# klutzy/suruga

Hardware: AMD Instinct MI355X
Metric: GiB/s device-resident ChaCha20-Poly1305 over 16 KiB TLS records, 1/2/4/8 GPUs (higher is better)
Workload: dtype u32

## Files before the change

suruga_amd/csrc/sg_msg.hip:

```cpp
#include "sg_internal.h"
#include "sg_msg_plan.h"

#include "sg_device.h"

namespace sg {
namespace {

using namespace dev;

constexpr uint32_t kLdsFront = 64;
constexpr uint32_t kLdsBytes = kLdsFront + 64u + kMsgTileBytes + 16u;

struct MsgKey {
    uint32_t k[8];
    uint32_t r0, r1, r2, r3;
    uint32_t s[4];
};

__device__ __forceinline__ MsgKey msg_key(const uint8_t* key, uint32_t n14, uint32_t n15) {
    MsgKey mk;
#pragma unroll
    for (int i = 0; i < 8; ++i)
        mk.k[i] = uniform((uint32_t)key[4 * i] | ((uint32_t)key[4 * i + 1] << 8) | ((uint32_t)key[4 * i + 2] << 16) |
                          ((uint32_t)key[4 * i + 3] << 24));
    uint32_t ks[16];
    chacha_block(ks, mk.k, 0u, n14, n15);
    mk.r0 = uniform(ks[0] & 0x0fffffffu);
    mk.r1 = uniform(ks[1] & 0x0ffffffcu);
    mk.r2 = uniform(ks[2] & 0x0ffffffcu);
    mk.r3 = uniform(ks[3] & 0x0ffffffcu);
#pragma unroll
    for (int i = 0; i < 4; ++i) mk.s[i] = uniform(ks[4 + i]);
    return mk;
}

__device__ __forceinline__ F26 fpow(const F26 x, const uint32_t e) {
    F26 acc = f26_one();
    if (e == 0u) return acc;
    for (int bit = 31 - __builtin_clz(e); bit >= 0; --bit) {
        acc = fmul(acc, acc);
        if ((e >> bit) & 1u) acc = fmul(acc, x);
    }
    return acc;
}

__device__ __forceinline__ F26 block_sum(const F26 x, uint32_t* red, const uint32_t lane) {
    store_f26(red + 5u * lane, x);
    __syncthreads();
    if (lane < 16u) {
        F26 a = f26_zero();
        for (uint32_t i = 0; i < 16u; ++i) a = f26_add(a, load_f26(red + 5u * (16u * lane + i)));
        store_f26(red + 5u * (256u + lane), carry1(a));
    }
    __syncthreads();
    F26 a = f26_zero();
    if (lane == 0u) {
        for (uint32_t i = 0; i < 16u; ++i) a = f26_add(a, load_f26(red + 5u * (256u + i)));
        a = carry1(a);
    }
    return a;
}

}

struct MsgParams {
    const uint8_t* key;
    const uint8_t* ad;
    const uint8_t* in;
    uint8_t* out;
    uint8_t* status;
    uint32_t* ws;
    uint64_t n, adlen;
    uint32_t n14, n15;
    sg_msg_plan plan;
};

namespace {

template <bool OPEN>
__global__ __launch_bounds__(256) void sg_msg_kernel(const MsgParams p) {
    __shared__ __attribute__((aligned(64))) uint8_t lds[kLdsBytes];
    static_assert(kLdsBytes >= 5u * 4u * (256u + 16u), "reduction space");
    const uint32_t lane = threadIdx.x;
    const MsgKey mk = msg_key(p.key, p.n14, p.n15);
    const uint32_t r0 = mk.r0, r1 = mk.r1, r2 = mk.r2, r3 = mk.r3;
    const uint32_t s1 = r1 + (r1 >> 2), s2 = r2 + (r2 >> 2), s3 = r3 + (r3 >> 2);
    const F26 r = words_to_f26(r0, r1, r2, r3, 0u);
    const F26 R = fpow(r, p.plan.tile_blocks);
    const F26 Pl = fpow(r, lane < kMsgMacLanes ? kMsgLaneBlocks * (kMsgMacLanes - 1u - lane) : 0u);
    const ChaChaPre pre = chacha_pre(mk.k, p.n14, p.n15);

    const int64_t n = (int64_t)p.n;
    const int64_t adlen = (int64_t)p.adlen;
    const int64_t P = adlen + 8;
    const int64_t L = P + n + 8;
    const int64_t TB = (int64_t)p.plan.tile_bytes;
    const uint64_t z = p.plan.zero_blocks;
    const uint64_t last = z + p.plan.mac_blocks - 1u;
    const uint32_t rem = (uint32_t)(L - 16 * ((int64_t)p.plan.mac_blocks - 1));

    const uint64_t t0 = (uint64_t)blockIdx.x * p.plan.tiles_per_group;
    uint64_t t1 = t0 + p.plan.tiles_per_group;
    if (t1 > p.plan.tiles) t1 = p.plan.tiles;

    F26 acc = f26_zero();
    for (uint64_t t = t0; t < t1; ++t) {
        const int64_t s0 = (int64_t)t * TB - 16 * (int64_t)z;
        const int64_t s1e = s0 + TB;
        const int64_t d0 = s0 - P > 0 ? s0 - P : 0;
        const int64_t d1 = s1e - P < n ? s1e - P : n;
        const uint32_t A = (uint32_t)((s0 - P) & 63);
        uint8_t* tl = lds + kLdsFront + A;

        if (d1 > d0) {
            const int64_t cb = (d0 >> 6) + (int64_t)lane;
            const int64_t boff = cb << 6;
            if (boff < d1) {
                const uint8_t* ip = p.in + boff;
                uint8_t* op = p.out + boff;
                uint8_t* lp = tl + (P + boff - s0);
                const bool al = ((((uintptr_t)ip) | ((uintptr_t)op)) & 15u) == 0u;
                const bool full = al && boff >= d0 && boff + 64 <= d1;
                u32x4 dv[4] = {};
                bool vec[4] = {full, full, full, full};
                if (full) {
#pragma unroll
                    for (int c = 0; c < 4; ++c) dv[c] = gld16(ip + 16 * c);
                } else {
#pragma unroll
                    for (int c = 0; c < 4; ++c) {
                        const int64_t co = boff + 16 * c;
                        vec[c] = al && co + 16 > d0 && co < d1 && co + 16 <= n;
                        if (vec[c]) dv[c] = gld16(ip + 16 * c);
                    }
                }
                uint32_t ks[16];
                chacha_block_pre(ks, pre, mk.k, (uint32_t)cb + 1u, p.n14, p.n15);
                if (full) {
                    u32x4 xv[4];
#pragma unroll
                    for (int c = 0; c < 4; ++c) {
                        xv[c] = dv[c] ^ u32x4{ks[4 * c], ks[4 * c + 1], ks[4 * c + 2], ks[4 * c + 3]};
                        asm volatile("" : "+v"(xv[c].x), "+v"(xv[c].y), "+v"(xv[c].z), "+v"(xv[c].w));
                    }
#pragma unroll
                    for (int c = 0; c < 4; ++c) st16(lp + 16 * c, OPEN ? dv[c] : xv[c]);
#pragma unroll
                    for (int c = 0; c < 4; ++c) gst16(op + 16 * c, xv[c]);
                } else {
#pragma unroll
                for (int c = 0; c < 4; ++c) {
                    const int64_t co = boff + 16 * c;
                    if (co + 16 <= d0 || co >= d1) continue;
                    if (vec[c]) {
                        const u32x4 d = dv[c];
                        const u32x4 x = d ^ u32x4{ks[4 * c], ks[4 * c + 1], ks[4 * c + 2], ks[4 * c + 3]};
                        st16(lp + 16 * c, OPEN ? d : x);
                        if (co >= d0 && co + 16 <= d1) {
                            gst16(op + 16 * c, x);
                        } else {
                            const uint32_t xw[4] = {x.x, x.y, x.z, x.w};
#pragma unroll
                            for (int b = 0; b < 16; ++b)
                                if (co + b >= d0 && co + b < d1) op[16 * c + b] = (uint8_t)(xw[b >> 2] >> (8 * (b & 3)));
                        }
                    } else {
                        uint8_t xb[16];
#pragma unroll
                        for (int b = 0; b < 16; ++b) xb[b] = co + b >= d0 && co + b < d1 ? ip[16 * c + b] : (uint8_t)0;
#pragma unroll
                        for (int b = 0; b < 16; ++b) {
                            if (co + b >= d0 && co + b < d1) {
                                const uint8_t y = xb[b] ^ (uint8_t)(ks[4 * c + (b >> 2)] >> (8 * (b & 3)));
                                op[16 * c + b] = y;
                                lp[16 * c + b] = OPEN ? xb[b] : y;
                            }
                        }
                    }
                }
                }
            }
        }
        if (s0 < P || s1e > P + n) {
            int64_t a = s0 > 0 ? s0 : 0, b = s1e < P ? s1e : P;
            for (int64_t s = a + lane; s < b; s += kMsgThreads)
                tl[s - s0] = s < adlen ? p.ad[s] : (uint8_t)((uint64_t)adlen >> (8 * (s - adlen)));
            a = s0 > P + n ? s0 : P + n;
            for (int64_t s = a + lane; s < s1e; s += kMsgThreads) {
                const int64_t i = s - (P + n);
                tl[s - s0] = i < 8 ? (uint8_t)((uint64_t)n >> (8 * i)) : (uint8_t)0;
            }
        }
        __syncthreads();

        if (lane < kMsgMacLanes) {
            const uint64_t vb0 = t * p.plan.tile_blocks + kMsgLaneBlocks * lane;
            const uint8_t* bp = tl + 16u * kMsgLaneBlocks * lane;
            H32 h = {0u, 0u, 0u, 0u, 0u};
#pragma unroll
            for (uint32_t j = 0; j < kMsgLaneBlocks; ++j) {
                u32x4 m = ldu16(bp + 16u * j);
                const uint64_t vb = vb0 + j;
                uint32_t pad = 1u;
                if (vb < z) {
                    m = u32x4{0u, 0u, 0u, 0u};
                    pad = 0u;
                } else if (vb == last && rem < 16u) {
                    const uint32_t fb = 1u << (8u * (rem & 3u));
                    const uint32_t fw = rem >> 2;
                    m.x |= fw == 0u ? fb : 0u;
                    m.y |= fw == 1u ? fb : 0u;
                    m.z |= fw == 2u ? fb : 0u;
                    m.w |= fw == 3u ? fb : 0u;
                    pad = 0u;
                }
                horner_step(h, m.x, m.y, m.z, m.w, pad, r0, r1, r2, r3, s1, s2, s3);
            }
            F26 f = words_to_f26(h.h0, h.h1, h.h2, h.h3, 0u);
            f.v4 += h.h4 << 24;
            const uint32_t c = f.v4 >> 26;
            f.v4 &= M26;
            f.v0 += c * 5u;
            acc = fmul_add(acc, R, f);
        }
        __syncthreads();
    }
    const F26 Hg = block_sum(fmul(acc, Pl), reinterpret_cast<uint32_t*>(lds), lane);
    if (lane == 0u) store_f26(p.ws + (uint64_t)blockIdx.x * kMsgPartialWords, Hg);
}

template <bool OPEN>
__global__ __launch_bounds__(256) void sg_msg_finish_kernel(const MsgParams p) {
    __shared__ uint32_t red[5u * (256u + 16u)];
    const uint32_t lane = threadIdx.x;
    const MsgKey mk = msg_key(p.key, p.n14, p.n15);
    const F26 R = fpow(words_to_f26(mk.r0, mk.r1, mk.r2, mk.r3, 0u), p.plan.tile_blocks);
    F26 sum = f26_zero();
    for (uint32_t g = lane; g < p.plan.groups; g += 256u) {
        const uint64_t done = (uint64_t)(g + 1u) * p.plan.tiles_per_group;
        const uint32_t after = done >= p.plan.tiles ? 0u : (uint32_t)(p.plan.tiles - done);
        sum = f26_add(sum, fmul(load_f26(p.ws + (uint64_t)g * kMsgPartialWords), fpow(R, after)));
    }
    const F26 total = block_sum(carry1(sum), red, lane);
    if (lane != 0u) return;
    uint32_t tw[4];
    tag_words(total, mk.s, tw);
    if constexpr (!OPEN) {
        uint8_t* tp = p.out + p.n;
#pragma unroll
        for (int i = 0; i < 16; ++i) tp[i] = (uint8_t)(tw[i >> 2] >> (8 * (i & 3)));
    } else {
        const uint8_t* ep = p.in + p.n;
        uint32_t diff = 0u;
#pragma unroll
        for (int i = 0; i < 16; ++i) diff |= (uint32_t)ep[i] ^ ((tw[i >> 2] >> (8 * (i & 3))) & 0xffu);
        *p.status = diff != 0u ? 1u : 0u;
    }
}

__global__ __launch_bounds__(256) void sg_msg_scrub_kernel(uint8_t* out, const uint64_t n, const uint8_t* status) {
    if (*status == 0u) return;
    uint64_t head = (16u - ((uintptr_t)out & 15u)) & 15u;
    if (head > n) head = n;
    const uint64_t nvec = (n - head) >> 4;
    const uint64_t tail0 = head + (nvec << 4);
    const uint64_t i = (uint64_t)blockIdx.x * 256u + threadIdx.x;
    const uint64_t stride = (uint64_t)gridDim.x * 256u;
    for (uint64_t v = i; v < nvec; v += stride) st16(out + head + (v << 4), u32x4{0u, 0u, 0u, 0u});
    if (i < head) out[i] = 0;
    if (i < n - tail0) out[tail0 + i] = 0;
}

}

hipError_t launch_msg(const uint8_t* key, const uint8_t nonce[8], const uint8_t* ad, uint64_t adlen, const uint8_t* in,
                      uint8_t* out, uint64_t n, uint8_t* status, uint32_t* ws, const sg_msg_plan& plan, bool open,
                      bool scrub, hipStream_t s) {
    if (plan.tile_blocks != kMsgTileBlocks || plan.groups == 0u || plan.groups > kMsgMaxGroups)
        return hipErrorInvalidValue;
    MsgParams p;
    p.key = key;
    p.ad = ad;
    p.in = in;
    p.out = out;
    p.status = status;
    p.ws = ws;
    p.n = n;
    p.adlen = adlen;
    p.n14 = (uint32_t)nonce[0] | ((uint32_t)nonce[1] << 8) | ((uint32_t)nonce[2] << 16) | ((uint32_t)nonce[3] << 24);
    p.n15 = (uint32_t)nonce[4] | ((uint32_t)nonce[5] << 8) | ((uint32_t)nonce[6] << 16) | ((uint32_t)nonce[7] << 24);
    p.plan = plan;
    if (open) {
        hipLaunchKernelGGL((sg_msg_kernel<true>), dim3(plan.groups), dim3(kMsgThreads), 0, s, p);
        hipLaunchKernelGGL((sg_msg_finish_kernel<true>), dim3(1), dim3(256), 0, s, p);
        if (scrub && n) {
            const uint64_t blocks = (n / 16u + 1023u) / 1024u;
            const uint32_t grid = blocks < 1u ? 1u : (blocks > 4096u ? 4096u : (uint32_t)blocks);
            hipLaunchKernelGGL(sg_msg_scrub_kernel, dim3(grid), dim3(256), 0, s, out, n, (const uint8_t*)status);
        }
    } else {
        hipLaunchKernelGGL((sg_msg_kernel<false>), dim3(plan.groups), dim3(kMsgThreads), 0, s, p);
        hipLaunchKernelGGL((sg_msg_finish_kernel<false>), dim3(1), dim3(256), 0, s, p);
    }
    return hipGetLastError();
}

}
```

Before: 2141.

## Double-buffer message tiles with buffer-resource loads and prefetch next span

Restructures the fused ChaCha20/Poly1305 message kernel so that each tile's input is prefetched into registers during the previous tile. It uses raw buffer loads and stores with out-of-range offsets to mask edges branch-free, and double-buffers LDS so only one barrier per tile is needed. Edge bytes are staged through a small LDS array, and an aligned/unaligned template split is chosen on the host. It also computes lane powers of r by square-and-multiply with a single shared R, skips the padding logic in interior tiles, and simplifies the finish-kernel power computation. The cost is more complexity and more LDS, and the single-barrier scheme and buffer-resource bounds tricks carry correctness risk.

```diff
diff --git a/suruga_amd/csrc/sg_msg.hip b/suruga_amd/csrc/sg_msg.hip
--- a/suruga_amd/csrc/sg_msg.hip
+++ b/suruga_amd/csrc/sg_msg.hip
@@ -10,6 +10,7 @@
 
 constexpr uint32_t kLdsFront = 64;
 constexpr uint32_t kLdsBytes = kLdsFront + 64u + kMsgTileBytes + 16u;
+constexpr uint32_t kLdsBuf = (kLdsBytes + 63u) & ~63u;
 
 struct MsgKey {
     uint32_t k[8];
@@ -77,17 +78,111 @@
 
 namespace {
 
-template <bool OPEN>
+constexpr uint32_t kSpanBytes = 64u * kMsgThreads;
+constexpr uint32_t kNoChunk = 0x7ffffff0u;
+typedef uint32_t bufv4 __attribute__((vector_size(16)));
+
+__device__ __forceinline__ __amdgpu_buffer_rsrc_t span_rsrc(const uint8_t* base) {
+    return __builtin_amdgcn_make_buffer_rsrc(const_cast<uint8_t*>(base), 0, (int)kSpanBytes, 0x00020000);
+}
+__device__ __forceinline__ u32x4 bld16(__amdgpu_buffer_rsrc_t rs, uint32_t off) {
+    const bufv4 v = __builtin_amdgcn_raw_buffer_load_b128(rs, (int)off, 0, 0);
+    return u32x4{v[0], v[1], v[2], v[3]};
+}
+__device__ __forceinline__ void bst16(__amdgpu_buffer_rsrc_t rs, uint32_t off, u32x4 v) {
+    __builtin_amdgcn_raw_buffer_store_b128(bufv4{v.x, v.y, v.z, v.w}, rs, (int)off, 0, 0);
+}
+
+__device__ __forceinline__ void tile_barrier() { asm volatile("s_waitcnt lgkmcnt(0)\n\ts_barrier" ::: "memory"); }
+
+struct Span {
+    int64_t base;
+    uint32_t r0, r1;
+    uint32_t rn;
+    uint32_t lofs;
+};
+
+struct Chunks {
+    bool whole[4];
+    bool edge[4];
+    bool ld[4];
+};
+__device__ __forceinline__ Chunks chunks_of(const Span& sp, const uint32_t lane) {
+    Chunks ch;
+#pragma unroll
+    for (uint32_t c = 0; c < 4u; ++c) {
+        const uint32_t rel = 64u * lane + 16u * c;
+        ch.whole[c] = rel >= sp.r0 && rel + 16u <= sp.r1;
+        ch.edge[c] = !ch.whole[c] && rel + 16u > sp.r0 && rel < sp.r1;
+        ch.ld[c] = ch.whole[c] || (ch.edge[c] && rel + 16u <= sp.rn);
+    }
+    return ch;
+}
+
+template <bool SPECIAL>
+__device__ __forceinline__ F26 lane_mac(const uint8_t* bp, const uint64_t vb0, const uint64_t z, const uint64_t last,
+                                        const uint32_t rem, const uint32_t r0, const uint32_t r1, const uint32_t r2,
+                                        const uint32_t r3, const uint32_t s1, const uint32_t s2, const uint32_t s3) {
+    H32 h = {0u, 0u, 0u, 0u, 0u};
+#pragma unroll
+    for (uint32_t j = 0; j < kMsgLaneBlocks; ++j) {
+        u32x4 m = ldu16(bp + 16u * j);
+        uint32_t pad = 1u;
+        if constexpr (SPECIAL) {
+            const uint64_t vb = vb0 + j;
+            if (vb < z) {
+                m = u32x4{0u, 0u, 0u, 0u};
+                pad = 0u;
+            } else if (vb == last && rem < 16u) {
+                const uint32_t fb = 1u << (8u * (rem & 3u));
+                const uint32_t fw = rem >> 2;
+                m.x |= fw == 0u ? fb : 0u;
+                m.y |= fw == 1u ? fb : 0u;
+                m.z |= fw == 2u ? fb : 0u;
+                m.w |= fw == 3u ? fb : 0u;
+                pad = 0u;
+            }
+        }
+        horner_step(h, m.x, m.y, m.z, m.w, pad, r0, r1, r2, r3, s1, s2, s3);
+    }
+    F26 f = words_to_f26(h.h0, h.h1, h.h2, h.h3, 0u);
+    f.v4 += h.h4 << 24;
+    const uint32_t c = f.v4 >> 26;
+    f.v4 &= M26;
+    f.v0 += c * 5u;
+    return f;
+}
+
+template <bool OPEN, bool AL>
 __global__ __launch_bounds__(256) void sg_msg_kernel(const MsgParams p) {
-    __shared__ __attribute__((aligned(64))) uint8_t lds[kLdsBytes];
-    static_assert(kLdsBytes >= 5u * 4u * (256u + 16u), "reduction space");
+    __shared__ __attribute__((aligned(64))) uint8_t lds[2u * kLdsBuf];
+    __shared__ __attribute__((aligned(16))) uint8_t edge[2][16];
+    __shared__ uint32_t xch[5];
+    static_assert(kLdsBuf >= 5u * 4u * (256u + 16u), "reduction space");
     const uint32_t lane = threadIdx.x;
     const MsgKey mk = msg_key(p.key, p.n14, p.n15);
-    const uint32_t r0 = mk.r0, r1 = mk.r1, r2 = mk.r2, r3 = mk.r3;
-    const uint32_t s1 = r1 + (r1 >> 2), s2 = r2 + (r2 >> 2), s3 = r3 + (r3 >> 2);
+    uint32_t r0 = mk.r0, r1 = mk.r1, r2 = mk.r2, r3 = mk.r3;
+    uint32_t s1 = r1 + (r1 >> 2), s2 = r2 + (r2 >> 2), s3 = r3 + (r3 >> 2);
     const F26 r = words_to_f26(r0, r1, r2, r3, 0u);
-    const F26 R = fpow(r, p.plan.tile_blocks);
-    const F26 Pl = fpow(r, lane < kMsgMacLanes ? kMsgLaneBlocks * (kMsgMacLanes - 1u - lane) : 0u);
+    asm volatile("" : "+v"(r0), "+v"(r1), "+v"(r2), "+v"(r3), "+v"(s1), "+v"(s2), "+v"(s3));
+    const F26 rr = fmul(r, r);
+    const F26 r4 = fmul(rr, rr);
+    F26 Pl = f26_one();
+    {
+        const uint32_t e = lane < kMsgMacLanes ? kMsgMacLanes - 1u - lane : 0u;
+        F26 q = r4;
+#pragma unroll
+        for (uint32_t k = 0; k < 8u; ++k) {
+            const bool on = (e >> k) & 1u;
+            const F26 m = {on ? q.v0 : 1u, on ? q.v1 : 0u, on ? q.v2 : 0u, on ? q.v3 : 0u, on ? q.v4 : 0u};
+            Pl = fmul(Pl, m);
+            if (k < 7u) q = fmul(q, q);
+        }
+    }
+    if (lane == 0u) store_f26(xch, Pl);
+    __syncthreads();
+    F26 R = fmul(load_f26(xch), r4);
+    asm volatile("" : "+v"(R.v0), "+v"(R.v1), "+v"(R.v2), "+v"(R.v3), "+v"(R.v4));
     const ChaChaPre pre = chacha_pre(mk.k, p.n14, p.n15);
 
     const int64_t n = (int64_t)p.n;
@@ -98,86 +193,120 @@
     const uint64_t z = p.plan.zero_blocks;
     const uint64_t last = z + p.plan.mac_blocks - 1u;
     const uint32_t rem = (uint32_t)(L - 16 * ((int64_t)p.plan.mac_blocks - 1));
+    const uint32_t A = (uint32_t)((-16 * (int64_t)z - P) & 63);
 
     const uint64_t t0 = (uint64_t)blockIdx.x * p.plan.tiles_per_group;
     uint64_t t1 = t0 + p.plan.tiles_per_group;
     if (t1 > p.plan.tiles) t1 = p.plan.tiles;
+
+    auto span_of = [&](const uint64_t t) {
+        Span sp = {0, 0u, 0u, 0u, 0u};
+        if (t >= t1) return sp;
+        const int64_t s0 = (int64_t)t * TB - 16 * (int64_t)z;
+        const int64_t d0 = s0 - P > 0 ? s0 - P : 0;
+        const int64_t d1 = s0 + TB - P < n ? s0 + TB - P : n;
+        if (d1 <= d0) return sp;
+        sp.base = d0 & ~(int64_t)63;
+        sp.r0 = (uint32_t)(d0 - sp.base);
+        sp.r1 = (uint32_t)(d1 - sp.base);
+        sp.rn = n - sp.base < (int64_t)(1u << 30) ? (uint32_t)(n - sp.base) : (1u << 30);
+        sp.lofs = kLdsFront + A + (uint32_t)(P + sp.base - s0);
+        return sp;
+    };
+
+    Span sp = span_of(t0);
+    u32x4 dv[4] = {};
+    if constexpr (AL) {
+        const Chunks ch = chunks_of(sp, lane);
+        const __amdgpu_buffer_rsrc_t ri = span_rsrc(p.in + sp.base);
+#pragma unroll
+        for (uint32_t c = 0; c < 4u; ++c) dv[c] = bld16(ri, ch.ld[c] ? 64u * lane + 16u * c : kNoChunk);
+#pragma unroll
+        for (uint32_t c = 0; c < 4u; ++c) bst16(ri, kNoChunk - 16u * c, u32x4{0u, 0u, 0u, 0u});
+    }
 
     F26 acc = f26_zero();
     for (uint64_t t = t0; t < t1; ++t) {
         const int64_t s0 = (int64_t)t * TB - 16 * (int64_t)z;
         const int64_t s1e = s0 + TB;
-        const int64_t d0 = s0 - P > 0 ? s0 - P : 0;
-        const int64_t d1 = s1e - P < n ? s1e - P : n;
-        const uint32_t A = (uint32_t)((s0 - P) & 63);
-        uint8_t* tl = lds + kLdsFront + A;
-
-        if (d1 > d0) {
-            const int64_t cb = (d0 >> 6) + (int64_t)lane;
-            const int64_t boff = cb << 6;
-            if (boff < d1) {
+        uint8_t* buf = lds + (uint32_t)(t & 1u) * kLdsBuf;
+        uint8_t* tl = buf + kLdsFront + A;
+        const Span nx = span_of(t + 1u);
+
+        if constexpr (AL) {
+            const Chunks ch = chunks_of(sp, lane);
+            uint32_t ks[16];
+            chacha_block_pre(ks, pre, mk.k, (uint32_t)(sp.base >> 6) + lane + 1u, p.n14, p.n15);
+            uint8_t* lp = buf + sp.lofs + 64u * lane;
+            u32x4 xv[4];
+#pragma unroll
+            for (uint32_t c = 0; c < 4u; ++c) {
+                const u32x4 kv = u32x4{ks[4 * c], ks[4 * c + 1], ks[4 * c + 2], ks[4 * c + 3]};
+                xv[c] = dv[c] ^ kv;
+                if (ch.ld[c]) st16(lp + 16u * c, OPEN ? dv[c] : xv[c]);
+                if (ch.edge[c]) st16(edge[64u * lane + 16u * c < sp.r0 ? 0 : 1], ch.ld[c] ? xv[c] : kv);
+            }
+            {
+                const Chunks cn = chunks_of(nx, lane);
+                const __amdgpu_buffer_rsrc_t ri = span_rsrc(p.in + nx.base);
+#pragma unroll
+                for (uint32_t c = 0; c < 4u; ++c) dv[c] = bld16(ri, cn.ld[c] ? 64u * lane + 16u * c : kNoChunk);
+            }
+            const __amdgpu_buffer_rsrc_t ro = span_rsrc(p.out + sp.base);
+#pragma unroll
+            for (uint32_t c = 0; c < 4u; ++c) bst16(ro, ch.whole[c] ? 64u * lane + 16u * c : kNoChunk, xv[c]);
+
+            const uint32_t cf = sp.r0 & ~15u, cbk = sp.r1 & ~15u;
+            const bool front = (sp.r0 & 15u) != 0u && sp.r1 > sp.r0;
+            const bool back = (sp.r1 & 15u) != 0u && sp.r1 > sp.r0 && !(front && cbk == cf);
+            const uint32_t wave = uniform(lane >> 6);
+            const bool mine_f = front && wave == 0u, mine_b = back && wave == (cbk >> 12);
+            if (mine_f || mine_b) {
+                wave_lds_sync();
+                const uint32_t e = (lane >> 4) & 1u, j = lane & 15u;
+                const uint32_t crel = e ? cbk : cf;
+                const uint32_t rel = crel + j;
+                const bool on = (lane & 63u) < 32u && (e ? mine_b : mine_f) && rel >= sp.r0 && rel < sp.r1;
+                const bool tail_f = mine_f && cf + 16u > sp.rn, tail_b = mine_b && cbk + 16u > sp.rn;
+                if (!(tail_f || tail_b)) {
+                    if (on) p.out[sp.base + rel] = edge[e][j];
+                } else {
+                    if (on) {
+                        const bool staged = crel + 16u <= sp.rn;
+                        uint8_t y = edge[e][j];
+                        if (!staged) {
+                            const uint8_t x = p.in[sp.base + rel];
+                            y ^= x;
+                            buf[sp.lofs + rel] = OPEN ? x : y;
+                        }
+                        p.out[sp.base + rel] = y;
+                    }
+                }
+            }
+        } else {
+            const int64_t d0 = sp.base + sp.r0, d1 = sp.base + sp.r1;
+            const int64_t boff = sp.base + 64 * (int64_t)lane;
+            if (d1 > d0 && boff < d1) {
                 const uint8_t* ip = p.in + boff;
                 uint8_t* op = p.out + boff;
-                uint8_t* lp = tl + (P + boff - s0);
-                const bool al = ((((uintptr_t)ip) | ((uintptr_t)op)) & 15u) == 0u;
-                const bool full = al && boff >= d0 && boff + 64 <= d1;
-                u32x4 dv[4] = {};
-                bool vec[4] = {full, full, full, full};
-                if (full) {
-#pragma unroll
-                    for (int c = 0; c < 4; ++c) dv[c] = gld16(ip + 16 * c);
-                } else {
-#pragma unroll
-                    for (int c = 0; c < 4; ++c) {
-                        const int64_t co = boff + 16 * c;
-                        vec[c] = al && co + 16 > d0 && co < d1 && co + 16 <= n;
-                        if (vec[c]) dv[c] = gld16(ip + 16 * c);
-                    }
-                }
+                uint8_t* lp = buf + sp.lofs + 64u * lane;
                 uint32_t ks[16];
-                chacha_block_pre(ks, pre, mk.k, (uint32_t)cb + 1u, p.n14, p.n15);
-                if (full) {
-                    u32x4 xv[4];
-#pragma unroll
-                    for (int c = 0; c < 4; ++c) {
-                        xv[c] = dv[c] ^ u32x4{ks[4 * c], ks[4 * c + 1], ks[4 * c + 2], ks[4 * c + 3]};
-                        asm volatile("" : "+v"(xv[c].x), "+v"(xv[c].y), "+v"(xv[c].z), "+v"(xv[c].w));
-                    }
-#pragma unroll
-                    for (int c = 0; c < 4; ++c) st16(lp + 16 * c, OPEN ? dv[c] : xv[c]);
-#pragma unroll
-                    for (int c = 0; c < 4; ++c) gst16(op + 16 * c, xv[c]);
-                } else {
+                chacha_block_pre(ks, pre, mk.k, (uint32_t)(boff >> 6) + 1u, p.n14, p.n15);
 #pragma unroll
                 for (int c = 0; c < 4; ++c) {
                     const int64_t co = boff + 16 * c;
                     if (co + 16 <= d0 || co >= d1) continue;
-                    if (vec[c]) {
-                        const u32x4 d = dv[c];
-                        const u32x4 x = d ^ u32x4{ks[4 * c], ks[4 * c + 1], ks[4 * c + 2], ks[4 * c + 3]};
-                        st16(lp + 16 * c, OPEN ? d : x);
-                        if (co >= d0 && co + 16 <= d1) {
-                            gst16(op + 16 * c, x);
-                        } else {
-                            const uint32_t xw[4] = {x.x, x.y, x.z, x.w};
-#pragma unroll
-                            for (int b = 0; b < 16; ++b)
-                                if (co + b >= d0 && co + b < d1) op[16 * c + b] = (uint8_t)(xw[b >> 2] >> (8 * (b & 3)));
-                        }
-                    } else {
-                        uint8_t xb[16];
-#pragma unroll
-                        for (int b = 0; b < 16; ++b) xb[b] = co + b >= d0 && co + b < d1 ? ip[16 * c + b] : (uint8_t)0;
-#pragma unroll
-                        for (int b = 0; b < 16; ++b) {
-                            if (co + b >= d0 && co + b < d1) {
-                                const uint8_t y = xb[b] ^ (uint8_t)(ks[4 * c + (b >> 2)] >> (8 * (b & 3)));
-                                op[16 * c + b] = y;
-                                lp[16 * c + b] = OPEN ? xb[b] : y;
-                            }
+                    uint8_t xb[16];
+#pragma unroll
+                    for (int b = 0; b < 16; ++b) xb[b] = co + b >= d0 && co + b < d1 ? ip[16 * c + b] : (uint8_t)0;
+#pragma unroll
+                    for (int b = 0; b < 16; ++b) {
+                        if (co + b >= d0 && co + b < d1) {
+                            const uint8_t y = xb[b] ^ (uint8_t)(ks[4 * c + (b >> 2)] >> (8 * (b & 3)));
+                            op[16 * c + b] = y;
+                            lp[16 * c + b] = OPEN ? xb[b] : y;
                         }
                     }
-                }
                 }
             }
         }
@@ -191,40 +320,19 @@
                 tl[s - s0] = i < 8 ? (uint8_t)((uint64_t)n >> (8 * i)) : (uint8_t)0;
             }
         }
-        __syncthreads();
+        tile_barrier();
 
         if (lane < kMsgMacLanes) {
             const uint64_t vb0 = t * p.plan.tile_blocks + kMsgLaneBlocks * lane;
             const uint8_t* bp = tl + 16u * kMsgLaneBlocks * lane;
-            H32 h = {0u, 0u, 0u, 0u, 0u};
-#pragma unroll
-            for (uint32_t j = 0; j < kMsgLaneBlocks; ++j) {
-                u32x4 m = ldu16(bp + 16u * j);
-                const uint64_t vb = vb0 + j;
-                uint32_t pad = 1u;
-                if (vb < z) {
-                    m = u32x4{0u, 0u, 0u, 0u};
-                    pad = 0u;
-                } else if (vb == last && rem < 16u) {
-                    const uint32_t fb = 1u << (8u * (rem & 3u));
-                    const uint32_t fw = rem >> 2;
-                    m.x |= fw == 0u ? fb : 0u;
-                    m.y |= fw == 1u ? fb : 0u;
-                    m.z |= fw == 2u ? fb : 0u;
-                    m.w |= fw == 3u ? fb : 0u;
-                    pad = 0u;
-                }
-                horner_step(h, m.x, m.y, m.z, m.w, pad, r0, r1, r2, r3, s1, s2, s3);
-            }
-            F26 f = words_to_f26(h.h0, h.h1, h.h2, h.h3, 0u);
-            f.v4 += h.h4 << 24;
-            const uint32_t c = f.v4 >> 26;
-            f.v4 &= M26;
-            f.v0 += c * 5u;
+            const bool special = t == 0u || t + 1u == p.plan.tiles;
+            const F26 f = special ? lane_mac<true>(bp, vb0, z, last, rem, r0, r1, r2, r3, s1, s2, s3)
+                                  : lane_mac<false>(bp, vb0, z, last, rem, r0, r1, r2, r3, s1, s2, s3);
             acc = fmul_add(acc, R, f);
         }
-        __syncthreads();
-    }
+        sp = nx;
+    }
+    __syncthreads();
     const F26 Hg = block_sum(fmul(acc, Pl), reinterpret_cast<uint32_t*>(lds), lane);
     if (lane == 0u) store_f26(p.ws + (uint64_t)blockIdx.x * kMsgPartialWords, Hg);
 }
@@ -235,12 +343,15 @@
     const uint32_t lane = threadIdx.x;
     const MsgKey mk = msg_key(p.key, p.n14, p.n15);
     const F26 R = fpow(words_to_f26(mk.r0, mk.r1, mk.r2, mk.r3, 0u), p.plan.tile_blocks);
+    const uint32_t G = p.plan.groups, per = p.plan.tiles_per_group;
+    const uint32_t a0 = (uint32_t)(p.plan.tiles - (uint64_t)(G - 1u) * per);
+    const F26 Q = fpow(R, per);
+    const F26 Ra0 = fpow(R, a0);
     F26 sum = f26_zero();
-    for (uint32_t g = lane; g < p.plan.groups; g += 256u) {
-        const uint64_t done = (uint64_t)(g + 1u) * p.plan.tiles_per_group;
-        const uint32_t after = done >= p.plan.tiles ? 0u : (uint32_t)(p.plan.tiles - done);
-        sum = f26_add(sum, fmul(load_f26(p.ws + (uint64_t)g * kMsgPartialWords), fpow(R, after)));
-    }
+    for (uint32_t g = lane; g + 1u < G; g += 256u)
+        sum = f26_add(sum, fmul(load_f26(p.ws + (uint64_t)g * kMsgPartialWords), fpow(Q, G - 2u - g)));
+    sum = fmul(carry1(sum), Ra0);
+    if (lane == ((G - 1u) & 255u)) sum = f26_add(sum, load_f26(p.ws + (uint64_t)(G - 1u) * kMsgPartialWords));
     const F26 total = block_sum(carry1(sum), red, lane);
     if (lane != 0u) return;
     uint32_t tw[4];
@@ -290,16 +401,20 @@
     p.n14 = (uint32_t)nonce[0] | ((uint32_t)nonce[1] << 8) | ((uint32_t)nonce[2] << 16) | ((uint32_t)nonce[3] << 24);
     p.n15 = (uint32_t)nonce[4] | ((uint32_t)nonce[5] << 8) | ((uint32_t)nonce[6] << 16) | ((uint32_t)nonce[7] << 24);
     p.plan = plan;
+    const bool al = ((((uintptr_t)in) | ((uintptr_t)out)) & 15u) == 0u;
+    const dim3 grid(plan.groups), block(kMsgThreads);
     if (open) {
-        hipLaunchKernelGGL((sg_msg_kernel<true>), dim3(plan.groups), dim3(kMsgThreads), 0, s, p);
+        if (al) hipLaunchKernelGGL((sg_msg_kernel<true, true>), grid, block, 0, s, p);
+        else hipLaunchKernelGGL((sg_msg_kernel<true, false>), grid, block, 0, s, p);
         hipLaunchKernelGGL((sg_msg_finish_kernel<true>), dim3(1), dim3(256), 0, s, p);
         if (scrub && n) {
             const uint64_t blocks = (n / 16u + 1023u) / 1024u;
-            const uint32_t grid = blocks < 1u ? 1u : (blocks > 4096u ? 4096u : (uint32_t)blocks);
-            hipLaunchKernelGGL(sg_msg_scrub_kernel, dim3(grid), dim3(256), 0, s, out, n, (const uint8_t*)status);
+            const uint32_t sgrid = blocks < 1u ? 1u : (blocks > 4096u ? 4096u : (uint32_t)blocks);
+            hipLaunchKernelGGL(sg_msg_scrub_kernel, dim3(sgrid), dim3(256), 0, s, out, n, (const uint8_t*)status);
         }
     } else {
-        hipLaunchKernelGGL((sg_msg_kernel<false>), dim3(plan.groups), dim3(kMsgThreads), 0, s, p);
+        if (al) hipLaunchKernelGGL((sg_msg_kernel<false, true>), grid, block, 0, s, p);
+        else hipLaunchKernelGGL((sg_msg_kernel<false, false>), grid, block, 0, s, p);
         hipLaunchKernelGGL((sg_msg_finish_kernel<false>), dim3(1), dim3(256), 0, s, p);
     }
     return hipGetLastError();
```

Result: no change. 2142 (median of 2 runs) (+0.0%).
